# yxtay/glove-tensorflow

Hardware: AMD Instinct MI355X
Metric: co-occurrence nonzeros/sec (higher is better)
Workload: dtype f32; 1 GPU; zipf_v400k_d300; V=400000, d=300, optimizer=Adagrad, batch_size_per_gpu=1048576, global_batch=1048576, nnz_per_gpu=25000000, chunk_cap=32, parallelism=single GPU, index=dealt

## Files before the change

### glove-tensorflow_amd/csrc/glove_epoch.hip

```cpp
#include "glove_common.h"

#include <type_traits>

namespace glove {

constexpr int kCsThreads = 256;
constexpr int kCsWaves = kCsThreads / 64;
constexpr int kCsMaxDigits = 2048;
constexpr int kCsMaxBits = 11;

struct CsGeom {
    int64_t n;
    int ntiles;
    int nd[2], db[2];
    int stride;
    uint32_t *count, *offs;
    uint32_t *tot;
};

template <int E, class Job>
__global__ __launch_bounds__(kCsThreads) void csort_hist(Job job, CsGeom g)
{
    __shared__ int hist[kCsMaxDigits];
    const int side = blockIdx.y, nd = g.nd[side], db = g.db[side];
    for (int i = threadIdx.x; i < nd; i += kCsThreads) hist[i] = 0;
    __syncthreads();
    const int lane = threadIdx.x & 63, wave = threadIdx.x >> 6;
    const int64_t base = ((int64_t)blockIdx.x * kCsWaves + wave) * (64 * E);
    __shared__ uint32_t walk[Job::kSeats ? E * kCsThreads : 1];
    if (Job::kSeats) {
        int cnt = 0;
#pragma unroll
        for (int j = 0; j < E; ++j) {
            const int64_t i = base + j * 64 + lane;
            if (i < g.n) { walk[j * kCsThreads + threadIdx.x] = job.position(side, i); cnt = j + 1; }
        }
        int j = 0;
        uint32_t x = cnt > 0 ? walk[threadIdx.x] : 0u;
        while (j < cnt) {
            x = job.seat_once(x);
            if (job.seated(x)) {
                walk[j * kCsThreads + threadIdx.x] = x;
                ++j;
                if (j < cnt) x = walk[j * kCsThreads + threadIdx.x];
            }
        }
    }
#pragma unroll 4
    for (int j = 0; j < E; ++j) {
        const int64_t i = base + j * 64 + lane;
        const bool valid = i < g.n;
        int digit = 0;
        if (Job::kSeats) { if (valid) digit = job.digit_of_seat(side, i, walk[j * kCsThreads + threadIdx.x]); }
        else if (valid) digit = job.digit(side, i);
        const unsigned long long peers = digit_peers(digit, db, valid);
        if (valid && lane == __ffsll((long long)peers) - 1) atomicAdd(&hist[digit], __popcll(peers));
    }
    __syncthreads();
    uint32_t *out = g.count + (size_t)side * g.stride * g.ntiles + blockIdx.x;
    for (int i = threadIdx.x; i < nd; i += kCsThreads) out[(size_t)i * g.ntiles] = (uint32_t)hist[i];
}

__device__ inline int block_excl_scan(int v, int *wtot , int &total)
{
    const int lane = threadIdx.x & 63, wave = threadIdx.x >> 6;
    int incl = v;
#pragma unroll
    for (int dlt = 1; dlt < 64; dlt <<= 1) {
        const int o = __shfl_up(incl, dlt, 64);
        if (lane >= dlt) incl += o;
    }
    __syncthreads();
    if (lane == 63) wtot[wave] = incl;
    __syncthreads();
    int start = incl - v;
    total = 0;
#pragma unroll
    for (int wv = 0; wv < kCsWaves; ++wv) {
        if (wv < wave) start += wtot[wv];
        total += wtot[wv];
    }
    return start;
}

__global__ __launch_bounds__(kCsThreads) void csort_scan(CsGeom g)
{
    __shared__ int wtot[kCsWaves];
    const int side = blockIdx.y, d = blockIdx.x;
    if (d >= g.nd[side]) return;
    const uint32_t *row = g.count + ((size_t)side * g.stride + d) * g.ntiles;
    uint32_t *out = g.offs + ((size_t)side * g.stride + d) * g.ntiles;
    constexpr int kPer = 8;
    int carry = 0;
    for (int base = 0; base < g.ntiles; base += kCsThreads * kPer) {
        int v[kPer], s = 0;
#pragma unroll
        for (int k = 0; k < kPer; ++k) {
            const int t = base + threadIdx.x * kPer + k;
            v[k] = t < g.ntiles ? (int)row[t] : 0;
            s += v[k];
        }
        int total;
        int run = carry + block_excl_scan(s, wtot, total);
#pragma unroll
        for (int k = 0; k < kPer; ++k) {
            const int t = base + threadIdx.x * kPer + k;
            if (t < g.ntiles) out[t] = (uint32_t)run;
            run += v[k];
        }
        carry += total;
    }
    if (threadIdx.x == 0) g.tot[(size_t)side * g.stride + d] = (uint32_t)carry;
}

template <int E, class Job>
__global__ __launch_bounds__(kCsThreads) void csort_scatter(Job job, CsGeom g)
{
    using Item = typename Job::Item;
    constexpr int T = kCsThreads * E;
    extern __shared__ __attribute__((aligned(16))) unsigned char cs_smem[];
    const int side = blockIdx.y, nd = g.nd[side], db = g.db[side];
    Item *stage = reinterpret_cast<Item *>(cs_smem);
    uint16_t *sdig = reinterpret_cast<uint16_t *>(stage + T);
    int *wcnt = reinterpret_cast<int *>(sdig + T);
    int *gbase = wcnt + kCsWaves * nd;
    int *tstart = gbase + nd;
    __shared__ int wtot[kCsWaves];
    const int lane = threadIdx.x & 63, wave = threadIdx.x >> 6;
    const int64_t tile0 = (int64_t)blockIdx.x * T;
    const int64_t base = tile0 + (int64_t)wave * (64 * E);
    Item it[E];
    int digit[E], rank[E];
#pragma unroll
    for (int j = 0; j < E; ++j) {
        const int64_t i = base + j * 64 + lane;
        digit[j] = 0;
        if (i < g.n) digit[j] = job.load(side, i, it[j]);
    }
    int *mine = wcnt + wave * nd;
    for (int i = lane; i < nd; i += 64) mine[i] = 0;
#pragma unroll
    for (int j = 0; j < E; ++j) {
// ... 443 lines not shown
```

### glove-tensorflow_amd/csrc/glove_plan.hip

```cpp
#include "glove_common.h"

#include <cstring>

namespace glove {

constexpr int kSmallPlanMax = 4096;
int plan_build_small(const int32_t *row, const int32_t *col, const float *w, const float *y, int64_t B, int32_t V,
                     const PlanSet &set, int n, hipStream_t st);

constexpr int kSortThreads = 256;
constexpr int kSortWaves = kSortThreads / 64;
constexpr int kMaxDigits = 256;
constexpr int kWalk = 16;

struct SortSide {
    const int32_t *keys;
    const int32_t *vals;
    int32_t clean_below;
    int32_t *out_keys, *out_vals;
    int32_t *sorted_keys;
    const int32_t *other;
    int32_t other_below;
    int32_t *partner;
    float *w_out, *y_out;
    int32_t *where;
};

struct SortPass {
    SortSide s[2];
    const float *w, *y;
    int4 *pairs;
    int64_t n;
    int shift, db;
    int ntiles;
    uint16_t *count;
    int tile_stride;
    int32_t *mapped;
};

__device__ inline void block_store_sum(int v, int32_t *out)
{
    __shared__ int part[kSortWaves];
    v = wave_sum_int(v);
    if ((threadIdx.x & 63) == 0) part[threadIdx.x >> 6] = v;
    __syncthreads();
    if (threadIdx.x == 0) {
        int s = 0;
        for (int wv = 0; wv < kSortWaves; ++wv) s += part[wv];
        *out = s;
    }
}

template <int E>
__device__ inline void sort_load_keys(const SortSide &sd, int64_t n, int64_t base, int32_t (&key)[E], int &mapped)
{
    const int lane = threadIdx.x & 63;
#pragma unroll
    for (int j = 0; j < E; ++j) {
        const int64_t i = base + j * 64 + lane;
        int32_t k = 0;
        if (i < n) {
            k = sd.keys[i];
            if (sd.clean_below > 0 && (uint32_t)k >= (uint32_t)sd.clean_below) { k = 0; ++mapped; }
        }
        key[j] = k;
    }
}

struct SortPassSet { SortPass b[kPlanSetMax]; };
__device__ inline const SortPass &pick(const SortPass &a) { return a; }
__device__ inline const SortPass &pick(const SortPassSet &a) { return a.b[blockIdx.z]; }

template <int E, class Args>
__global__ __launch_bounds__(kSortThreads) void radix_hist(Args args)
{
    const SortPass &in = pick(args);
    static_assert(kSortThreads == kMaxDigits, "one thread per digit zeroes and stores the histogram");
    __shared__ int hist[kMaxDigits];
    const int side = blockIdx.y;
    const SortSide &sd = in.s[side];
    const int nd = 1 << in.db, lane = threadIdx.x & 63, wave = threadIdx.x >> 6;
    hist[threadIdx.x] = 0;
    __syncthreads();
    const int64_t base = ((int64_t)blockIdx.x * kSortWaves + wave) * (64 * E);
// ... 72 lines not shown
    int all = 0, earlier = 0;
    const int me = blockIdx.x;
    for (int q0 = 0; q0 < nq; q0 += kWalk) {
        if (q0 > 0) {
#pragma unroll
            for (int x = 0; x < kWalk; ++x) cw[x] = rowp[q0 + x < nq ? q0 + x : 0];
        }
#pragma unroll
        for (int x = 0; x < kWalk; ++x) {
            const uint32_t wd[4] = {cw[x].x, cw[x].y, cw[x].z, cw[x].w};
#pragma unroll
            for (int h = 0; h < 8; ++h) {
                const int t = (q0 + x) * 8 + h;
                const int c = (int)((wd[h >> 1] >> (16 * (h & 1))) & 0xffffu);
                all += (q0 + x < nq && t < in.ntiles) ? c : 0;
                earlier += (q0 + x < nq && t < me) ? c : 0;
            }
        }
    }
    if ((int)threadIdx.x >= nd) all = earlier = 0;
    int incl = all;
#pragma unroll
    for (int dlt = 1; dlt < 64; dlt <<= 1) {
        const int o = __shfl_up(incl, dlt, 64);
        if (lane >= dlt) incl += o;
    }
    if (lane == 63) scan_red[wave] = incl;
    __syncthreads();
    int start = incl - all + earlier;
    for (int wv = 0; wv < wave; ++wv) start += scan_red[wv];
    if ((int)threadIdx.x < nd) {
        int run = start;
#pragma unroll
        for (int wv = 0; wv < kSortWaves; ++wv) {
            const int c = wcnt[wv][threadIdx.x];
            wcnt[wv][threadIdx.x] = run;
            run += c;
        }
    }
    __syncthreads();
#pragma unroll
    for (int j = 0; j < E; ++j) {
        const int64_t i = base + j * 64 + lane;
        if (i >= in.n) continue;
        const int digit = (key[j] >> in.shift) & (nd - 1);
        const int dest = wcnt[wave][digit] + rank[j];
        const int32_t p = val[j];
        if (!LAST) {
            sd.out_keys[dest] = key[j];
            sd.out_vals[dest] = p;
        } else {
            sd.sorted_keys[dest] = key[j];
            int32_t o = g_id[j];
            if ((uint32_t)o >= (uint32_t)sd.other_below) o = 0;
            sd.partner[dest] = o;
            sd.w_out[dest] = g_w[j];
            sd.y_out[dest] = g_y[j];
            if (sd.where) { if (side == 0) sd.where[p] = dest; else sd.where[dest] = p; }
        }
    }
}


#define SIDE(x) (side ? x[1] : x[0])

constexpr int kTileThreads = 256;
constexpr int kTilePer = 8;
constexpr int kTile = kTileThreads * kTilePer;

struct SideKeys { const int32_t *keys[2]; };
struct SideOut {
    int32_t *chunk_id[2], *chunk_start[2], *uniq_slot[2];
    int32_t *counts;
    int32_t *uniq_rec[2];
    const int64_t *tile_re;
    int32_t *heavy;
    int heavy_chunks, cap_heavy;
    int2 *chunk_aux[2];
    uint32_t *mark[2];
    int mark_words[2];
    uint32_t *chunk_hw[2];
};

__device__ inline void tile_flags(const int32_t *__restrict__ keys, int64_t B, int64_t begin, int32_t chunk_cap,
                                  int64_t first_run_start, unsigned (&flag)[kTilePer], int &nu, int &nc, int64_t *lds_rs)
{
    const int64_t k0 = begin + (int64_t)threadIdx.x * kTilePer;
    int32_t key[kTilePer + 1];
    key[0] = (k0 > 0 && k0 <= B) ? keys[k0 - 1] : -1;
#pragma unroll
    for (int i = 0; i < kTilePer; ++i) key[i + 1] = (k0 + i < B) ? keys[k0 + i] : -1;
    int64_t my_last_start = -1;
#pragma unroll
    for (int i = 0; i < kTilePer; ++i) {
        const int64_t k = k0 + i;
        if (k < B && (k == 0 || key[i + 1] != key[i])) my_last_start = k;
    }
    const int lane = threadIdx.x & 63, wave = threadIdx.x >> 6;
    int64_t incl = my_last_start;
#pragma unroll
    for (int dlt = 1; dlt < 64; dlt <<= 1) {
        const int64_t o = __shfl_up(incl, dlt, 64);
        if (lane >= dlt) incl = o > incl ? o : incl;
    }
    if (lane == 63) lds_rs[wave] = incl;
    __syncthreads();
    int64_t carry = first_run_start;
    for (int wv = 0; wv < wave; ++wv) carry = lds_rs[wv] > carry ? lds_rs[wv] : carry;
    int64_t prev = __shfl_up(incl, 1, 64);
    if (lane == 0) prev = -1;
    int64_t run_start = prev > carry ? prev : carry;
    __syncthreads();
    nu = nc = 0;
#pragma unroll
    for (int i = 0; i < kTilePer; ++i) {
        const int64_t k = k0 + i;
        flag[i] = 0;
        if (k >= B) continue;
        const bool uniq = (k == 0 || key[i + 1] != key[i]);
        if (uniq) run_start = k;
        const bool chunk = uniq || ((int)(k - run_start) % chunk_cap == 0);
        flag[i] = (chunk ? 1u : 0u) | (uniq ? 2u : 0u);
        nu += uniq;
        nc += chunk;
    }
}

__device__ inline int64_t run_start_of(const int32_t *__restrict__ keys, int64_t pos)
{
    const int lane = threadIdx.x & 63;
    const int32_t key = keys[pos];
    int64_t lo = 0, hi = pos;
    if (pos > 0) {
        const int64_t q = pos - 1 - lane;
        const bool other = q >= 0 && keys[q] != key;
        const unsigned long long m = __ballot(other);
        if (m != 0) return pos - (__ffsll((long long)m) - 1);
        if (pos < 64) return 0;
        hi = pos - 64;
    }
    while (lo < hi) {
        const int64_t n = hi - lo, step = (n + 63) / 64;
        int64_t q = lo + step * lane;
        if (q > hi - 1) q = hi - 1;
        const bool ge = keys[q] >= key;
        const unsigned long long m = __ballot(ge);
        if (m == 0) {
            lo = __shfl(q, 63, 64) + 1;
            continue;
        }
        const int first = __ffsll((long long)m) - 1;
        const int64_t q_first = __shfl(q, first, 64);
        const int64_t q_before = __shfl(q, first > 0 ? first - 1 : 0, 64);
        lo = first == 0 ? lo : q_before + 1;
        hi = first == 0 ? lo : q_first;
    }
    return lo;
}

__device__ inline int64_t run_end_of(const int32_t *__restrict__ keys, int64_t B, int64_t pos)
{
    const int lane = threadIdx.x & 63;
    const int32_t key = keys[pos];
    int64_t lo = pos + 1, hi = B;
    {
        const int64_t q = pos + 1 + lane;
        const bool other = q < B && keys[q] != key;
        const unsigned long long m = __ballot(other);
        if (m != 0) return pos + 1 + (__ffsll((long long)m) - 1);
        if (pos + 65 >= B) return B;
        lo = pos + 65;
    }
    while (lo < hi) {
        const int64_t n = hi - lo, step = (n + 63) / 64;
        int64_t q = lo + step * lane;
        if (q > hi - 1) q = hi - 1;
        const bool gt = keys[q] > key;
        const unsigned long long m = __ballot(gt);
        if (m == 0) {
            lo = __shfl(q, 63, 64) + 1;
            continue;
        }
        const int first = __ffsll((long long)m) - 1;
        const int64_t q_first = __shfl(q, first, 64);
        const int64_t q_before = __shfl(q, first > 0 ? first - 1 : 0, 64);
        lo = first == 0 ? lo : q_before + 1;
        hi = first == 0 ? lo : q_first;
    }
    return lo;
}

struct TileExtra {
    int64_t *tile_re;
    int32_t *counts;
    const int32_t *mapped;
    int n_mapped;
    const int32_t *c_orig;
    const int32_t *rpos;
    int32_t *c_perm, *r_to_c;
};

struct SideCopy {
    const int32_t *p_src[2]; const float *w_src[2], *y_src[2];
    int32_t *p_dst[2]; float *w_dst[2], *y_dst[2];
};

struct SideOne {
    SideKeys sk;
    int64_t *tile_rs;
    int2 *tile_sums;
    TileExtra ex;
    SideOut out;
    SideCopy cp;
};
struct SideSet { SideOne b[kPlanSetMax]; };
__device__ inline const SideOne &pick(const SideOne &a) { return a; }
__device__ inline const SideOne &pick(const SideSet &a) { return a.b[blockIdx.z]; }

struct SortedSrc { const int32_t *id[2], *partner[2]; const float *w[2], *y[2]; };
struct SortedWs { char *base; size_t per_batch, tile_rs, tile_re, tile_sums, aux0, aux1; };
struct SideDev {
    const glove_plan *plans;
    SortedSrc src;
    SortedWs ws;
    int64_t B;
    int ntiles;
    int32_t V;
};
__device__ inline SideOne pick(const SideDev &a)
{
    const glove_plan &pl = a.plans[blockIdx.z];
    const size_t at = (size_t)blockIdx.z * (size_t)a.B;
    char *w = a.ws.base + (size_t)blockIdx.z * a.ws.per_batch;
    SideOne o;
    o.sk = SideKeys{{a.src.id[0] + at, a.src.id[1] + at}};
    o.tile_rs = reinterpret_cast<int64_t *>(w + a.ws.tile_rs);
    o.tile_sums = reinterpret_cast<int2 *>(w + a.ws.tile_sums);
    int64_t *tile_re = reinterpret_cast<int64_t *>(w + a.ws.tile_re);
    int2 *aux0 = reinterpret_cast<int2 *>(w + a.ws.aux0), *aux1 = reinterpret_cast<int2 *>(w + a.ws.aux1);
    o.ex = TileExtra{tile_re, pl.counts, nullptr, 0, nullptr, nullptr, nullptr, nullptr};
    o.out = SideOut{{pl.r_chunk_id, pl.c_chunk_id}, {pl.r_chunk_start, pl.c_chunk_start}, {pl.r_uniq_slot, pl.c_uniq_slot},
                    pl.counts, {pl.r_uniq_rec, pl.c_uniq_rec}, tile_re, pl.heavy, pl.heavy_chunks, pl.cap_heavy,
                    {pl.r_crec ? aux0 : nullptr, pl.r_crec ? aux1 : nullptr},
                    {pl.r_mark, pl.c_mark}, {((pl.V_row > 0 ? pl.V_row : a.V) + 31) / 32, (a.V + 31) / 32},
                    {pl.r_chunk_hw, pl.c_chunk_hw}};
    o.cp = SideCopy{{a.src.partner[0] + at, a.src.partner[1] + at}, {a.src.w[0] + at, a.src.w[1] + at}, {a.src.y[0] + at, a.src.y[1] + at},
                    {pl.r_partner, pl.c_partner}, {pl.r_w, pl.c_w}, {pl.r_y, pl.c_y}};
    return o;
}

template <class Args>
__global__ __launch_bounds__(kTileThreads) void side_tiles(Args args, int64_t B, int32_t chunk_cap, int ntiles)
{
    const SideOne &one = pick(args);
    const SideKeys &sk = one.sk;
    int64_t *__restrict__ tile_rs = one.tile_rs;
    int2 *__restrict__ tile_sums = one.tile_sums;
    const TileExtra &ex = one.ex;
    __shared__ int64_t lds_rs[kTileThreads / 64 + 1];
    __shared__ int red[2][kTileThreads / 64];
    const int side = blockIdx.y, t = blockIdx.x;
    const int32_t *keys = SIDE(sk.keys);
    const int64_t begin = (int64_t)t * kTile;
    if (SIDE(one.out.mark)) {
        uint32_t *mk = SIDE(one.out.mark);
        const int words = SIDE(one.out.mark_words);
        for (int i = t * kTileThreads + (int)threadIdx.x; i < words; i += ntiles * kTileThreads) mk[i] = 0u;
    }
    if (SIDE(one.cp.p_dst)) {
        const SideCopy &cp = one.cp;
        for (int64_t k = begin + threadIdx.x; k < begin + kTile && k < B; k += kTileThreads) {
            SIDE(cp.p_dst)[k] = SIDE(cp.p_src)[k];
            SIDE(cp.w_dst)[k] = SIDE(cp.w_src)[k];
            SIDE(cp.y_dst)[k] = SIDE(cp.y_src)[k];
        }
    }
    if (side == 1 && ex.c_perm) {
        const int64_t q0 = begin + (int64_t)threadIdx.x * kTilePer;
        int32_t o[kTilePer], rp[kTilePer];
#pragma unroll
        for (int i = 0; i < kTilePer; ++i) o[i] = q0 + i < B ? ex.c_orig[q0 + i] : 0;
#pragma unroll
        for (int i = 0; i < kTilePer; ++i) rp[i] = ex.rpos[o[i]];
#pragma unroll
        for (int i = 0; i < kTilePer; ++i) {
            if (q0 + i >= B) continue;
            ex.c_perm[q0 + i] = rp[i];
            ex.r_to_c[rp[i]] = (int32_t)(q0 + i);
        }
    }
    if (threadIdx.x < 64) {
        const int64_t r = begin > 0 ? run_start_of(keys, begin) : 0;
        if (threadIdx.x == 0) lds_rs[kTileThreads / 64] = r;
    } else if (threadIdx.x < 128) {
        const int64_t end = begin + kTile < B ? begin + kTile : B;
        const int64_t r = end < B ? run_end_of(keys, B, end - 1) : B;
        if (threadIdx.x == 64) ex.tile_re[(size_t)side * ntiles + t] = r;
    }
    __syncthreads();
    const int64_t frs = lds_rs[kTileThreads / 64];
    unsigned flag[kTilePer];
    int nu, nc;
    tile_flags(keys, B, begin, chunk_cap, frs, flag, nu, nc, lds_rs);
    nu = wave_sum_int(nu);
    nc = wave_sum_int(nc);
    if ((threadIdx.x & 63) == 0) { red[0][threadIdx.x >> 6] = nu; red[1][threadIdx.x >> 6] = nc; }
    __syncthreads();
    if (threadIdx.x == 0) {
        int su = 0, sc = 0;
        for (int wv = 0; wv < kTileThreads / 64; ++wv) { su += red[0][wv]; sc += red[1][wv]; }
        tile_sums[(size_t)side * ntiles + t] = make_int2(su, sc);
        tile_rs[(size_t)side * ntiles + t] = frs;
    }
    if (t == 0 && side == 0) {
        int v = 0;
        for (int i = threadIdx.x; i < ex.n_mapped; i += kTileThreads) v += ex.mapped[i];
        v = wave_sum_int(v);
        __syncthreads();
        if ((threadIdx.x & 63) == 0) red[0][threadIdx.x >> 6] = v;
        __syncthreads();
        if (threadIdx.x == 0) {
            int total = 0;
            for (int wv = 0; wv < kTileThreads / 64; ++wv) total += red[0][wv];
            ex.counts[5] = total;
            ex.counts[4] = ex.counts[6] = ex.counts[7] = 0;
        }
    }
}

template <class Args>
__global__ __launch_bounds__(kTileThreads) void side_emit(Args args, int64_t B, int32_t chunk_cap, int ntiles)
{
    const SideOne &one = pick(args);
    const SideKeys &sk = one.sk;
    const int64_t *__restrict__ tile_rs = one.tile_rs;
    const int2 *__restrict__ tile_sums = one.tile_sums;
    const SideOut &out = one.out;
    __shared__ int64_t lds_rs[kTileThreads / 64 + 1];
    __shared__ int64_t lds_open[kTileThreads / 64];
    __shared__ int red[2][kTileThreads / 64];
    __shared__ int wave_tot[2][kTileThreads / 64];
    const int side = blockIdx.y, t = blockIdx.x;
    const int32_t *keys = SIDE(sk.keys);
    const int64_t begin = (int64_t)t * kTile;
    int pu = 0, pc = 0;
    for (int i = threadIdx.x; i < t; i += kTileThreads) {
        const int2 v = tile_sums[(size_t)side * ntiles + i];
        pu += v.x;
        pc += v.y;
    }
    pu = wave_sum_int(pu);
    pc = wave_sum_int(pc);
    if ((threadIdx.x & 63) == 0) { red[0][threadIdx.x >> 6] = pu; red[1][threadIdx.x >> 6] = pc; }
    __syncthreads();
    int base_u = 0, base_c = 0;
    for (int wv = 0; wv < kTileThreads / 64; ++wv) { base_u += red[0][wv]; base_c += red[1][wv]; }
    unsigned flag[kTilePer];
    int nu, nc;
    tile_flags(keys, B, begin, chunk_cap, tile_rs[(size_t)side * ntiles + t], flag, nu, nc, lds_rs);
    const int lane = threadIdx.x & 63, wave = threadIdx.x >> 6;
    int iu = nu, ic = nc;
#pragma unroll
    for (int dlt = 1; dlt < 64; dlt <<= 1) {
        const int ou = __shfl_up(iu, dlt, 64), oc = __shfl_up(ic, dlt, 64);
        if (lane >= dlt) { iu += ou; ic += oc; }
    }
    if (lane == 63) { wave_tot[0][wave] = iu; wave_tot[1][wave] = ic; }
    __syncthreads();
    int ui = base_u + iu - nu, ci = base_c + ic - nc;
    for (int wv = 0; wv < wave; ++wv) { ui += wave_tot[0][wv]; ci += wave_tot[1][wv]; }
    const int64_t k0 = begin + (int64_t)threadIdx.x * kTilePer;
    int32_t *chunk_id = SIDE(out.chunk_id), *chunk_start = SIDE(out.chunk_start), *uniq_slot = SIDE(out.uniq_slot);
    int open_ui[kTilePer], open_ci[kTilePer];
    int64_t my_first_open = INT64_MAX;
#pragma unroll
    for (int i = kTilePer - 1; i >= 0; --i)
        if (flag[i] & 2u) my_first_open = k0 + i;
#pragma unroll
    for (int i = 0; i < kTilePer; ++i) {
        const int64_t k = k0 + i;
        open_ui[i] = ui;
        open_ci[i] = ci;
        if (flag[i] & 2u) uniq_slot[ui++] = ci;
        if (flag[i] & 1u) { chunk_id[ci] = keys[k]; chunk_start[ci] = (int32_t)k; ++ci; }
        if (k == B - 1) {
            chunk_start[ci] = (int32_t)B;
            uniq_slot[ui] = ci;
            out.counts[2 * side] = ci;
            out.counts[2 * side + 1] = ui;
        }
    }
    int64_t sfx = my_first_open;
#pragma unroll
    for (int dlt = 1; dlt < 64; dlt <<= 1) {
        const int64_t o = __shfl_down(sfx, dlt, 64);
        if (lane + dlt < 64) sfx = o < sfx ? o : sfx;
    }
    if (lane == 0) lds_open[wave] = sfx;
    __syncthreads();
    int64_t next_open = out.tile_re[(size_t)side * ntiles + t];
    for (int wv = kTileThreads / 64 - 1; wv > wave; --wv) next_open = lds_open[wv] < next_open ? lds_open[wv] : next_open;
    int64_t right = __shfl_down(sfx, 1, 64);
    if (lane == 63) right = INT64_MAX;
    next_open = right < next_open ? right : next_open;
    int2 *aux = SIDE(out.chunk_aux);
#pragma unroll
    for (int i = kTilePer - 1; i >= 0; --i) {
        if (!(flag[i] & 1u)) continue;
        const int64_t k = k0 + i;
        const int pairs = (int)(next_open - k), chunks = (pairs + chunk_cap - 1) / chunk_cap;
        if (aux || SIDE(out.chunk_hw)) {
            const bool opens = (flag[i] & 2u) != 0;
            const uint32_t hw = (uint32_t)(chunks - 1) | (opens ? 0x80000000u : 0u);
            if (aux) aux[open_ci[i]] = make_int2(opens ? open_ui[i] : open_ui[i] - 1, (int)hw);
            if (SIDE(out.chunk_hw)) SIDE(out.chunk_hw)[open_ci[i]] = hw;
        }
        if (!(flag[i] & 2u)) continue;
        reinterpret_cast<int4 *>(SIDE(out.uniq_rec))[open_ui[i]] = make_int4(keys[k], open_ci[i], chunks, pairs);
        if (SIDE(out.mark)) atomicOr(SIDE(out.mark) + (keys[k] >> 5), 1u << (keys[k] & 31));
        if (chunks > out.heavy_chunks) {
            const int slot = atomicAdd(out.counts + 4, 1);
            if (slot < out.cap_heavy) out.heavy[slot] = (side << 30) | open_ui[i];
        }
        next_open = k;
    }
}

struct RecordArgs {
    const int32_t *uniq_slot[2];
    const int32_t *chunk_id[2], *chunk_start[2], *partner[2];
    const float *w[2], *y[2];
    int32_t *crec[2];
    const int2 *chunk_aux[2];
    int header_in_record;
};
struct RecordOne { RecordArgs a; const int32_t *counts; };
struct RecordSet { RecordOne b[kPlanSetMax]; };
__device__ inline const RecordOne &pick(const RecordOne &a) { return a; }
__device__ inline const RecordOne &pick(const RecordSet &a) { return a.b[blockIdx.z]; }
struct RecordDev { SideDev d; };
__device__ inline RecordOne pick(const RecordDev &r)
{
    const SideDev &a = r.d;
    const glove_plan &pl = a.plans[blockIdx.z];
    const size_t at = (size_t)blockIdx.z * (size_t)a.B;
    char *w = a.ws.base + (size_t)blockIdx.z * a.ws.per_batch;
    RecordOne o;
    o.a = RecordArgs{{pl.r_uniq_slot, pl.c_uniq_slot}, {pl.r_chunk_id, pl.c_chunk_id}, {pl.r_chunk_start, pl.c_chunk_start},
                     {a.src.partner[0] + at, a.src.partner[1] + at}, {a.src.w[0] + at, a.src.w[1] + at}, {a.src.y[0] + at, a.src.y[1] + at},
                     {pl.r_crec, pl.c_crec},
                     {reinterpret_cast<const int2 *>(w + a.ws.aux0), reinterpret_cast<const int2 *>(w + a.ws.aux1)}, 0};
    o.counts = pl.counts;
    return o;
}

typedef int v4i_t __attribute__((ext_vector_type(4)));

template <class Args>
__global__ __launch_bounds__(kBlock) void fill_records(Args args, int capP, int nt)
{
    const RecordOne &rone = pick(args);
    const RecordArgs &a = rone.a;
    const int32_t *__restrict__ counts = rone.counts;
    const int side = blockIdx.y;
    const int n_chunks = counts[2 * side];
    const int32_t *chunk_id = SIDE(a.chunk_id), *chunk_start = SIDE(a.chunk_start), *partner = SIDE(a.partner);
    const float *w = SIDE(a.w), *y = SIDE(a.y);
    const int2 *aux = SIDE(a.chunk_aux);
    const int sq = rec_stride_q(capP);
    const int lane = threadIdx.x & 63, g = lane & 7, oct = lane >> 3;
    const int j0 = (int)((blockIdx.x * (kBlock / 64) + (threadIdx.x >> 6)) * 32);
    if (j0 >= n_chunks) return;
    const int jl = j0 + lane < n_chunks ? j0 + lane : n_chunks;
    const int cs = lane <= 32 ? chunk_start[jl] : 0;
    constexpr int kStage = 384;
    __shared__ int32_t st_p[kBlock / 64][kStage];
    __shared__ float st_w[kBlock / 64][kStage], st_y[kBlock / 64][kStage];
    const int wv = threadIdx.x >> 6;
    const int p0 = __shfl(cs, 0, 64);
    const int last = n_chunks - j0 < 32 ? n_chunks - j0 : 32;
    const int span = __shfl(cs, last, 64) - p0;
    const bool staged = span <= kStage;
    if (staged) {
        for (int i = lane; i < span; i += 64) {
            st_p[wv][i] = partner[p0 + i];
            st_w[wv][i] = w[p0 + i];
            st_y[wv][i] = y[p0 + i];
        }
    }
    int32_t cid = 0;
    int2 ax = make_int2(0, 0);
    if (lane < 32 && j0 + lane < n_chunks) {
        cid = chunk_id[j0 + lane];
        if (aux) {
            ax = aux[j0 + lane];
        } else if (a.header_in_record) {
            ax = *reinterpret_cast<const int2 *>(SIDE(a.crec) + (size_t)(j0 + lane) * sq * 4 + 2);
        } else {
            const int j = j0 + lane;
            const int32_t *slot = SIDE(a.uniq_slot);
            int lo = 0, hi = counts[2 * side + 1];
            while (hi - lo > 1) {
                const int mid = (lo + hi) >> 1;
                if (slot[mid] <= j) lo = mid; else hi = mid;
            }
            ax = make_int2(lo, (int)((uint32_t)(slot[lo + 1] - 1 - j) | (slot[lo] == j ? 0x80000000u : 0u)));
        }
    }
// ... 139 lines not shown
            SortPass &in = set.b[j];
            in = fin[j];
            for (int sd = 0; sd < 2; ++sd) {
                if (p > 0) {
                    in.s[sd].keys = pw[j].keys[sd][(p - 1) & 1];
                    in.s[sd].vals = pw[j].vals[sd][(p - 1) & 1];
                    in.s[sd].clean_below = 0;
                }
                in.s[sd].out_keys = pw[j].keys[sd][p & 1];
                in.s[sd].out_vals = pw[j].vals[sd][p & 1];
            }
            in.n = B;
            in.shift = p * db;
            in.db = db;
            in.ntiles = pw[j].sort_tiles;
            in.count = pw[j].count;
            in.tile_stride = pw[j].tile_stride;
            in.mapped = pw[j].mapped;
        }
        const dim3 grid(pw[0].sort_tiles, 2, nb);
        if (nb == 1) {
            hipLaunchKernelGGL((radix_hist<E, SortPass>), grid, dim3(kSortThreads), 0, st, set.b[0]);
            if (p < P - 1) hipLaunchKernelGGL((radix_scatter<E, false, SortPass>), grid, dim3(kSortThreads), 0, st, set.b[0]);
            else hipLaunchKernelGGL((radix_scatter<E, true, SortPass>), grid, dim3(kSortThreads), 0, st, set.b[0]);
        } else {
            hipLaunchKernelGGL((radix_hist<E, SortPassSet>), grid, dim3(kSortThreads), 0, st, set);
            if (p < P - 1) hipLaunchKernelGGL((radix_scatter<E, false, SortPassSet>), grid, dim3(kSortThreads), 0, st, set);
            else hipLaunchKernelGGL((radix_scatter<E, true, SortPassSet>), grid, dim3(kSortThreads), 0, st, set);
        }
    }
}

#define HIP_TRY(expr) do { hipError_t e_ = (expr); if (e_ != hipSuccess) return (int)e_; } while (0)

static int build_tiled_set(const int32_t *row, const int32_t *col, const float *w, const float *y, int64_t B, int32_t V,
                           const glove_plan *const *plans, int nb, void *ws, size_t ws_bytes, hipStream_t st)
{
    const size_t per = carve_plan_ws(nullptr, B).bytes;
    if (per * (size_t)nb > ws_bytes) return GLOVE_E_WORKSPACE;
    PlanWs pw[kPlanSetMax];
    SortPass fin[kPlanSetMax];
    const int bits = ceil_log2(V);
    for (int j = 0; j < nb; ++j) {
        const glove_plan *plan = plans[j];
        pw[j] = carve_plan_ws((char *)ws + per * j, B);
        const int32_t Vr = plan->V_row > 0 ? plan->V_row : V;
        const size_t off = (size_t)j * B;
        SortPass &f = fin[j];
        f = SortPass{};
        f.w = w + off; f.y = y + off; f.pairs = pw[j].pairs;
        SortSide &rs = f.s[0], &cs = f.s[1];
        rs.keys = row + off; rs.vals = nullptr; rs.clean_below = Vr;
        rs.sorted_keys = pw[j].row_sorted; rs.other = col + off; rs.other_below = V;
        rs.partner = plan->r_partner; rs.w_out = plan->r_w; rs.y_out = plan->r_y; rs.where = plan->c_perm ? pw[j].rpos : nullptr;
        cs.keys = col + off; cs.vals = nullptr; cs.clean_below = V;
        cs.sorted_keys = pw[j].col_sorted; cs.other = row + off; cs.other_below = Vr;
        cs.partner = plan->c_partner; cs.w_out = plan->c_w; cs.y_out = plan->c_y; cs.where = plan->c_perm ? pw[j].c_orig : nullptr;
    }
    if (pw[0].sort_e == 4) launch_sorts<4>(fin, pw, nb, B, bits, st);
    else if (pw[0].sort_e == 8) launch_sorts<8>(fin, pw, nb, B, bits, st);
    else launch_sorts<16>(fin, pw, nb, B, bits, st);

    SideSet ss;
    const int2 *aux_r[kPlanSetMax], *aux_c[kPlanSetMax];
    for (int j = 0; j < nb; ++j) {
        const glove_plan *plan = plans[j];
        ss.b[j].sk = SideKeys{{pw[j].row_sorted, pw[j].col_sorted}};
        ss.b[j].tile_rs = pw[j].tile_rs;
        ss.b[j].tile_sums = pw[j].tile_sums;
        ss.b[j].out = SideOut{{plan->r_chunk_id, plan->c_chunk_id}, {plan->r_chunk_start, plan->c_chunk_start},
                            {plan->r_uniq_slot, plan->c_uniq_slot}, plan->counts, {plan->r_uniq_rec, plan->c_uniq_rec},
                            (const int64_t *)pw[j].tile_re, plan->heavy, plan->heavy_chunks, plan->cap_heavy,
                            {plan->r_crec ? pw[j].chunk_aux[0] : nullptr, plan->r_crec ? pw[j].chunk_aux[1] : nullptr},
                            {plan->r_mark, plan->c_mark}, {(Vr_of(plan, V) + 31) / 32, (V + 31) / 32},
                            {plan->r_chunk_hw, plan->c_chunk_hw}};
        ss.b[j].cp = SideCopy{};
        ss.b[j].ex = TileExtra{pw[j].tile_re, plan->counts, (const int32_t *)pw[j].mapped, 2 * pw[j].sort_tiles,
                             (const int32_t *)pw[j].c_orig, (const int32_t *)pw[j].rpos, plan->c_perm, plan->r_to_c};
        aux_r[j] = pw[j].chunk_aux[0];
        aux_c[j] = pw[j].chunk_aux[1];
    }
    const dim3 grid(pw[0].ntiles, 2, nb);
    if (nb == 1) {
        hipLaunchKernelGGL(side_tiles<SideOne>, grid, dim3(kTileThreads), 0, st, ss.b[0], B, plans[0]->chunk_cap, pw[0].ntiles);
        hipLaunchKernelGGL(side_emit<SideOne>, grid, dim3(kTileThreads), 0, st, ss.b[0], B, plans[0]->chunk_cap, pw[0].ntiles);
    } else {
        hipLaunchKernelGGL(side_tiles<SideSet>, grid, dim3(kTileThreads), 0, st, ss, B, plans[0]->chunk_cap, pw[0].ntiles);
        hipLaunchKernelGGL(side_emit<SideSet>, grid, dim3(kTileThreads), 0, st, ss, B, plans[0]->chunk_cap, pw[0].ntiles);
    }
    if (plans[0]->r_crec) return launch_fill_records_set(plans, nb, st, aux_r, aux_c);
    return (int)hipGetLastError();
}

}

using namespace glove;

extern "C" {

size_t glove_plan_workspace_bytes(int64_t B, int32_t V)
{
    (void)V;
    if (B < 0) return 0;
    return carve_plan_ws(nullptr, B).bytes;
}

static int check_plan_for_build(const glove_plan *plan, int64_t B, int32_t V)
{
    if (!plan->r_partner || !plan->r_w || !plan->r_y || !plan->r_chunk_id || !plan->r_chunk_start || !plan->r_uniq_slot ||
        !plan->c_w || !plan->c_y || !plan->r_uniq_rec || !plan->c_uniq_rec || !plan->c_partner || !plan->c_chunk_id || !plan->c_chunk_start || !plan->c_uniq_slot)
        return GLOVE_E_BADARG;
    if (!plan->heavy || plan->heavy_chunks < 1 ||
        plan->cap_heavy < 2 * B / ((int64_t)plan->heavy_chunks * plan->chunk_cap) + 2)
        return GLOVE_E_WORKSPACE;
    if (plan->cap_chunks < B || plan->cap_uniq < (B < V ? B : V)) return GLOVE_E_WORKSPACE;
    if ((plan->r_crec == nullptr) != (plan->c_crec == nullptr)) return GLOVE_E_BADARG;
    if ((plan->r_to_c == nullptr) != (plan->c_perm == nullptr)) return GLOVE_E_BADARG;
    if ((plan->r_mark == nullptr) != (plan->c_mark == nullptr)) return GLOVE_E_BADARG;
    if ((plan->r_chunk_hw == nullptr) != (plan->c_chunk_hw == nullptr)) return GLOVE_E_BADARG;
    return 0;
}

int glove_plan_build(const int32_t *row, const int32_t *col, const float *w, const float *y, int64_t B, int32_t V,
                     const glove_plan *plan, void *ws, size_t ws_bytes, void *stream)
{
    if (!plan || !ws || B < 0 || V <= 0 || plan->chunk_cap <= 0 || plan->B != B || !plan->counts) return GLOVE_E_BADARG;
    hipStream_t st = (hipStream_t)stream;
    if (B == 0) {
        HIP_TRY(zero_words(plan->counts, 8, st));
        return 0;
    }
    if (!row || !col || !w || !y) return GLOVE_E_BADARG;
    if (int rc = check_plan_for_build(plan, B, V)) return rc;
    if (B <= kSmallPlanMax) {
        PlanSet set;
        set.p[0] = *plan;
        if (int rc = plan_build_small(row, col, w, y, B, V, set, 1, st)) return rc;
        return plan->r_crec ? launch_fill_records(plan, st, true) : 0;
    }
    return build_tiled_set(row, col, w, y, B, V, &plan, 1, ws, ws_bytes, st);
}

static SortedWs carve_sorted_ws(void *ws, int64_t B, int *ntiles_out)
{
    SortedWs s;
    size_t off = 0;
    auto take = [&](size_t bytes) { const size_t q = off; off += align_up(bytes, 256); return q; };
    const size_t n = (size_t)(B > 0 ? B : 1);
    const int ntiles = (int)((n + kTile - 1) / kTile);
    s.base = (char *)ws;
    s.tile_rs = take((size_t)2 * ntiles * 8);
    s.tile_re = take((size_t)2 * ntiles * 8);
    s.tile_sums = take((size_t)2 * ntiles * 8);
    s.aux0 = take(n * 8);
    s.aux1 = take(n * 8);
    s.per_batch = off;
    if (ntiles_out) *ntiles_out = ntiles;
    return s;
}

size_t glove_plan_sorted_workspace_bytes(int64_t B, int32_t n_batches)
{
    if (B < 0 || n_batches < 0) return 0;
    return carve_sorted_ws(nullptr, B, nullptr).per_batch * (size_t)n_batches;
}

int32_t glove_plan_chunk_bound(int64_t B, int32_t cap_uniq, int32_t chunk_cap)
{
    if (B < 0 || cap_uniq < 0 || chunk_cap <= 0) return 0;
    const int64_t bound = (int64_t)cap_uniq + B / chunk_cap + 1;
    return (int32_t)(bound < B ? bound : B);
}

int glove_plan_build_sorted(const glove_pairs *row_side, const glove_pairs *col_side, int64_t first_pair, int64_t B,
                            int32_t n_batches, int32_t V, const glove_plan *plans, const glove_plan *plans_dev, void *ws,
                            size_t ws_bytes, void *stream)
{
    if (!row_side || !col_side || !plans || !plans_dev || first_pair < 0 || B <= 0 || n_batches < 0 || V <= 0) return GLOVE_E_BADARG;
    if (n_batches == 0) return 0;
    if (!row_side->id || !row_side->partner || !row_side->w || !row_side->y || !col_side->id || !col_side->partner || !col_side->w ||
        !col_side->y || !ws)
        return GLOVE_E_BADARG;
    int64_t most = 1;
    for (int j = 0; j < n_batches; ++j) {
        const glove_plan *p = plans + j;
        if (p->B != B || p->chunk_cap <= 0 || p->chunk_cap != plans[0].chunk_cap || !p->counts) return GLOVE_E_BADARG;
        if ((p->r_crec == nullptr) != (plans[0].r_crec == nullptr) || (p->r_crec == nullptr) != (p->c_crec == nullptr)) return GLOVE_E_BADARG;
        if (!p->r_chunk_id || !p->r_chunk_start || !p->r_uniq_slot || !p->r_uniq_rec || !p->c_chunk_id || !p->c_chunk_start ||
            !p->c_uniq_slot || !p->c_uniq_rec)
            return GLOVE_E_BADARG;
        const bool own = p->r_partner || p->r_w || p->r_y || p->c_partner || p->c_w || p->c_y;
        if (own && (!p->r_partner || !p->r_w || !p->r_y || !p->c_partner || !p->c_w || !p->c_y)) return GLOVE_E_BADARG;
        if (!own && !p->r_crec && !p->r_chunk_hw) return GLOVE_E_BADARG;
        if (p->c_perm || p->r_to_c) return GLOVE_E_BADARG;
        if ((p->r_mark == nullptr) != (p->c_mark == nullptr)) return GLOVE_E_BADARG;
        if ((p->r_chunk_hw == nullptr) != (p->c_chunk_hw == nullptr)) return GLOVE_E_BADARG;
        if (!p->heavy || p->heavy_chunks < 1 || p->cap_heavy < 2 * B / ((int64_t)p->heavy_chunks * p->chunk_cap) + 2) return GLOVE_E_WORKSPACE;
        if (p->cap_uniq < (B < V ? B : V)) return GLOVE_E_WORKSPACE;
        if (p->cap_chunks < glove_plan_chunk_bound(B, p->cap_uniq, p->chunk_cap)) return GLOVE_E_WORKSPACE;
        const int64_t mr = most_chunks(p, true), mc = most_chunks(p, false);
        most = mr > most ? mr : most;
        most = mc > most ? mc : most;
    }
    SideDev sd;
    sd.plans = plans_dev;
    sd.src = SortedSrc{{row_side->id + first_pair, col_side->id + first_pair}, {row_side->partner + first_pair, col_side->partner + first_pair},
                       {row_side->w + first_pair, col_side->w + first_pair}, {row_side->y + first_pair, col_side->y + first_pair}};
    sd.ws = carve_sorted_ws(ws, B, &sd.ntiles);
    sd.B = B;
    sd.V = V;
    if (sd.ws.per_batch * (size_t)n_batches > ws_bytes) return GLOVE_E_WORKSPACE;
    hipStream_t st = (hipStream_t)stream;
    const int32_t cap = plans[0].chunk_cap;
    for (int z0 = 0; z0 < n_batches; z0 += 65535) {
        const int nz = n_batches - z0 < 65535 ? n_batches - z0 : 65535;
        SideDev part = sd;
        part.plans = plans_dev + z0;
        part.ws.base = sd.ws.base + (size_t)z0 * sd.ws.per_batch;
        for (int x = 0; x < 2; ++x) {
            part.src.id[x] += (size_t)z0 * B; part.src.partner[x] += (size_t)z0 * B;
            part.src.w[x] += (size_t)z0 * B; part.src.y[x] += (size_t)z0 * B;
        }
        const dim3 grid(sd.ntiles, 2, nz);
        hipLaunchKernelGGL(side_tiles<SideDev>, grid, dim3(kTileThreads), 0, st, part, B, cap, sd.ntiles);
        hipLaunchKernelGGL(side_emit<SideDev>, grid, dim3(kTileThreads), 0, st, part, B, cap, sd.ntiles);
        if (plans[0].r_crec) {
            const int64_t per_block = (kBlock / 64) * 32;
            const int64_t nb = (most + per_block - 1) / per_block;
            hipLaunchKernelGGL(fill_records<RecordDev>, dim3((unsigned)(nb < 1 ? 1 : nb), 2, nz), dim3(kBlock), 0, st, RecordDev{part}, rec_cap(cap), B >= 262144 ? 1 : 0);
        }
    }
    return (int)hipGetLastError();
}

int glove_plan_fill_records(const glove_plan *plan, void *stream)
{
    if (!plan || !plan->r_crec || !plan->c_crec || !plan->counts || plan->chunk_cap <= 0) return GLOVE_E_BADARG;
    if (plan->B == 0) return 0;
    if (!plan->r_uniq_slot || !plan->c_uniq_slot) return GLOVE_E_BADARG;
    if (!plan->r_chunk_id || !plan->r_chunk_start || !plan->r_partner || !plan->r_w || !plan->r_y || !plan->c_chunk_id ||
        !plan->c_chunk_start || !plan->c_partner || !plan->c_w || !plan->c_y)
        return GLOVE_E_BADARG;
    return launch_fill_records(plan, (hipStream_t)stream);
}

}
```

Before: 1.866 billion nonzeros/s.

## Privatize small-radix histograms and streamline plan tile scan kernels

When a counting-sort pass has few digits, the histogram kernel now keeps 32 lane-indexed copies per digit in LDS and adds plain atomics to them, reducing them at the end instead of doing match-peer aggregation. The plan tile kernels load keys with 16-byte vector loads for full aligned tiles. They move run-start arithmetic to 32-bit tile-local offsets and replace the per-element modulo by chunk_cap with a running counter plus a precomputed magic-number divide. They also pack the unique and chunk counts into one int for a single wave reduction and scan, and drop a barrier by reordering the prefix-sum reads. The packing assumes per-tile counts fit in 16 bits, and the vector path adds a second template instantiation and more register pressure.

```diff
diff --git a/glove-tensorflow_amd/csrc/glove_epoch.hip b/glove-tensorflow_amd/csrc/glove_epoch.hip
--- a/glove-tensorflow_amd/csrc/glove_epoch.hip
+++ b/glove-tensorflow_amd/csrc/glove_epoch.hip
@@ -8,6 +8,9 @@
 constexpr int kCsWaves = kCsThreads / 64;
 constexpr int kCsMaxDigits = 2048;
 constexpr int kCsMaxBits = 11;
+constexpr int kCsFewDigits = 64;
+constexpr int kCsCopies = 32;
+static_assert(kCsFewDigits * kCsCopies <= kCsMaxDigits, "the copies share the histogram's LDS");
 
 struct CsGeom {
     int64_t n;
@@ -23,7 +26,8 @@
 {
     __shared__ int hist[kCsMaxDigits];
     const int side = blockIdx.y, nd = g.nd[side], db = g.db[side];
-    for (int i = threadIdx.x; i < nd; i += kCsThreads) hist[i] = 0;
+    const bool few = nd <= kCsFewDigits;
+    for (int i = threadIdx.x; i < (few ? nd * kCsCopies : nd); i += kCsThreads) hist[i] = 0;
     __syncthreads();
     const int lane = threadIdx.x & 63, wave = threadIdx.x >> 6;
     const int64_t base = ((int64_t)blockIdx.x * kCsWaves + wave) * (64 * E);
@@ -53,11 +57,28 @@
         int digit = 0;
         if (Job::kSeats) { if (valid) digit = job.digit_of_seat(side, i, walk[j * kCsThreads + threadIdx.x]); }
         else if (valid) digit = job.digit(side, i);
+        if (few) {
+            if (valid) atomicAdd(&hist[digit * kCsCopies + (lane & (kCsCopies - 1))], 1);
+            continue;
+        }
         const unsigned long long peers = digit_peers(digit, db, valid);
         if (valid && lane == __ffsll((long long)peers) - 1) atomicAdd(&hist[digit], __popcll(peers));
     }
     __syncthreads();
     uint32_t *out = g.count + (size_t)side * g.stride * g.ntiles + blockIdx.x;
+    if (few) {
+        static_assert(kCsFewDigits * 4 == kCsThreads && kCsCopies == 32, "four threads per digit, eight copies per thread");
+        const int d = threadIdx.x >> 2, part = threadIdx.x & 3;
+        int v = 0;
+        if (d < nd) {
+#pragma unroll
+            for (int r = 0; r < kCsCopies / 4; ++r) v += hist[d * kCsCopies + part * (kCsCopies / 4) + r];
+        }
+        v += __shfl_xor(v, 1, 64);
+        v += __shfl_xor(v, 2, 64);
+        if (d < nd && part == 0) out[(size_t)d * g.ntiles] = (uint32_t)v;
+        return;
+    }
     for (int i = threadIdx.x; i < nd; i += kCsThreads) out[(size_t)i * g.ntiles] = (uint32_t)hist[i];
 }
 
diff --git a/glove-tensorflow_amd/csrc/glove_plan.hip b/glove-tensorflow_amd/csrc/glove_plan.hip
--- a/glove-tensorflow_amd/csrc/glove_plan.hip
+++ b/glove-tensorflow_amd/csrc/glove_plan.hip
@@ -1,5 +1,6 @@
 #include "glove_common.h"
 
+#include <climits>
 #include <cstring>
 
 namespace glove {
@@ -238,47 +239,78 @@
     uint32_t *chunk_hw[2];
 };
 
-__device__ inline void tile_flags(const int32_t *__restrict__ keys, int64_t B, int64_t begin, int32_t chunk_cap,
-                                  int64_t first_run_start, unsigned (&flag)[kTilePer], int &nu, int &nc, int64_t *lds_rs)
-{
-    const int64_t k0 = begin + (int64_t)threadIdx.x * kTilePer;
-    int32_t key[kTilePer + 1];
-    key[0] = (k0 > 0 && k0 <= B) ? keys[k0 - 1] : -1;
-#pragma unroll
-    for (int i = 0; i < kTilePer; ++i) key[i + 1] = (k0 + i < B) ? keys[k0 + i] : -1;
-    int64_t my_last_start = -1;
+struct CapDiv { uint32_t m; int shift; };
+static CapDiv cap_div(int32_t d)
+{
+    int l = 0;
+    while ((1ll << l) < d) ++l;
+    const uint64_t p = 1ull << (31 + l);
+    return CapDiv{(uint32_t)((p + (uint64_t)d - 1) / (uint64_t)d), 31 + l};
+}
+__device__ inline int div_cap(int a, CapDiv cd) { return (int)(((uint64_t)(uint32_t)a * cd.m) >> cd.shift); }
+
+__device__ inline bool tile_whole(const int32_t *keys, int64_t B, int64_t begin)
+{
+    return begin + kTile <= B && (reinterpret_cast<uintptr_t>(keys + begin) & 15u) == 0;
+}
+
+template <bool WHOLE>
+__device__ inline void tile_keys(const int32_t *__restrict__ keys, int64_t B, int64_t k0, int32_t (&key)[kTilePer + 1])
+{
+    static_assert(kTilePer == 8, "two 16-byte loads per thread");
+    if (WHOLE) {
+        const int32_t front = keys[k0 > 0 ? k0 - 1 : 0];
+        const int4 a = *reinterpret_cast<const int4 *>(keys + k0), b = *reinterpret_cast<const int4 *>(keys + k0 + 4);
+        key[0] = k0 > 0 ? front : -1;
+        key[1] = a.x; key[2] = a.y; key[3] = a.z; key[4] = a.w;
+        key[5] = b.x; key[6] = b.y; key[7] = b.z; key[8] = b.w;
+    } else {
+        key[0] = (k0 > 0 && k0 <= B) ? keys[k0 - 1] : -1;
+#pragma unroll
+        for (int i = 0; i < kTilePer; ++i) key[i + 1] = (k0 + i < B) ? keys[k0 + i] : -1;
+    }
+}
+
+__device__ inline void tile_flags(const int32_t (&key)[kTilePer + 1], int64_t B, int64_t begin, int32_t chunk_cap, CapDiv cd,
+                                  int first_run_start, unsigned (&flag)[kTilePer], int &nu, int &nc, int *lds_rs)
+{
+    const int l0 = (int)threadIdx.x * kTilePer;
+    const int left = (int)(B - begin < kTile ? B - begin : kTile);
+    int my_last_start = INT_MIN;
 #pragma unroll
     for (int i = 0; i < kTilePer; ++i) {
-        const int64_t k = k0 + i;
-        if (k < B && (k == 0 || key[i + 1] != key[i])) my_last_start = k;
+        const int l = l0 + i;
+        if (l < left && ((begin == 0 && l == 0) || key[i + 1] != key[i])) my_last_start = l;
     }
     const int lane = threadIdx.x & 63, wave = threadIdx.x >> 6;
-    int64_t incl = my_last_start;
+    int incl = my_last_start;
 #pragma unroll
     for (int dlt = 1; dlt < 64; dlt <<= 1) {
-        const int64_t o = __shfl_up(incl, dlt, 64);
+        const int o = __shfl_up(incl, dlt, 64);
         if (lane >= dlt) incl = o > incl ? o : incl;
     }
     if (lane == 63) lds_rs[wave] = incl;
+    int prev = __shfl_up(incl, 1, 64);
+    if (lane == 0) prev = INT_MIN;
     __syncthreads();
-    int64_t carry = first_run_start;
+    int carry = first_run_start;
     for (int wv = 0; wv < wave; ++wv) carry = lds_rs[wv] > carry ? lds_rs[wv] : carry;
-    int64_t prev = __shfl_up(incl, 1, 64);
-    if (lane == 0) prev = -1;
-    int64_t run_start = prev > carry ? prev : carry;
-    __syncthreads();
+    int run_start = prev > carry ? prev : carry;
+    int behind = l0 < left ? l0 - run_start : 0;
+    behind -= div_cap(behind, cd) * chunk_cap;
     nu = nc = 0;
 #pragma unroll
     for (int i = 0; i < kTilePer; ++i) {
-        const int64_t k = k0 + i;
+        const int l = l0 + i;
         flag[i] = 0;
-        if (k >= B) continue;
-        const bool uniq = (k == 0 || key[i + 1] != key[i]);
-        if (uniq) run_start = k;
-        const bool chunk = uniq || ((int)(k - run_start) % chunk_cap == 0);
+        if (l >= left) continue;
+        const bool uniq = ((begin == 0 && l == 0) || key[i + 1] != key[i]);
+        if (uniq) behind = 0;
+        const bool chunk = behind == 0;
         flag[i] = (chunk ? 1u : 0u) | (uniq ? 2u : 0u);
         nu += uniq;
         nc += chunk;
+        if (++behind == chunk_cap) behind = 0;
     }
 }
 
@@ -405,19 +437,21 @@
     return o;
 }
 
-template <class Args>
-__global__ __launch_bounds__(kTileThreads) void side_tiles(Args args, int64_t B, int32_t chunk_cap, int ntiles)
-{
-    const SideOne &one = pick(args);
+template <bool WHOLE>
+__device__ inline void side_tiles_body(const SideOne &one, int64_t B, int32_t chunk_cap, CapDiv cd, int ntiles)
+{
     const SideKeys &sk = one.sk;
     int64_t *__restrict__ tile_rs = one.tile_rs;
     int2 *__restrict__ tile_sums = one.tile_sums;
     const TileExtra &ex = one.ex;
-    __shared__ int64_t lds_rs[kTileThreads / 64 + 1];
+    __shared__ int lds_rs[kTileThreads / 64];
+    __shared__ int64_t lds_frs;
     __shared__ int red[2][kTileThreads / 64];
     const int side = blockIdx.y, t = blockIdx.x;
     const int32_t *keys = SIDE(sk.keys);
     const int64_t begin = (int64_t)t * kTile;
+    int32_t key[kTilePer + 1];
+    tile_keys<WHOLE>(keys, B, begin + (int64_t)threadIdx.x * kTilePer, key);
     if (SIDE(one.out.mark)) {
         uint32_t *mk = SIDE(one.out.mark);
         const int words = SIDE(one.out.mark_words);
@@ -447,19 +481,20 @@
     }
     if (threadIdx.x < 64) {
         const int64_t r = begin > 0 ? run_start_of(keys, begin) : 0;
-        if (threadIdx.x == 0) lds_rs[kTileThreads / 64] = r;
+        if (threadIdx.x == 0) lds_frs = r;
     } else if (threadIdx.x < 128) {
         const int64_t end = begin + kTile < B ? begin + kTile : B;
         const int64_t r = end < B ? run_end_of(keys, B, end - 1) : B;
         if (threadIdx.x == 64) ex.tile_re[(size_t)side * ntiles + t] = r;
     }
     __syncthreads();
-    const int64_t frs = lds_rs[kTileThreads / 64];
+    const int64_t frs = lds_frs;
     unsigned flag[kTilePer];
     int nu, nc;
-    tile_flags(keys, B, begin, chunk_cap, frs, flag, nu, nc, lds_rs);
-    nu = wave_sum_int(nu);
-    nc = wave_sum_int(nc);
+    tile_flags(key, B, begin, chunk_cap, cd, (int)(frs - begin), flag, nu, nc, lds_rs);
+    nu = wave_sum_int(nu | nc << 16);
+    nc = nu >> 16;
+    nu &= 0xffff;
     if ((threadIdx.x & 63) == 0) { red[0][threadIdx.x >> 6] = nu; red[1][threadIdx.x >> 6] = nc; }
     __syncthreads();
     if (threadIdx.x == 0) {
@@ -485,22 +520,36 @@
 }
 
 template <class Args>
-__global__ __launch_bounds__(kTileThreads) void side_emit(Args args, int64_t B, int32_t chunk_cap, int ntiles)
+__global__ __launch_bounds__(kTileThreads) void side_tiles(Args args, int64_t B, int32_t chunk_cap, CapDiv cd, int ntiles)
 {
     const SideOne &one = pick(args);
+    const int side = blockIdx.y;
+    if (tile_whole(SIDE(one.sk.keys), B, (int64_t)blockIdx.x * kTile)) side_tiles_body<true>(one, B, chunk_cap, cd, ntiles);
+    else side_tiles_body<false>(one, B, chunk_cap, cd, ntiles);
+}
+
+template <bool WHOLE>
+__device__ inline void side_emit_body(const SideOne &one, int64_t B, int32_t chunk_cap, CapDiv cd, int ntiles)
+{
     const SideKeys &sk = one.sk;
     const int64_t *__restrict__ tile_rs = one.tile_rs;
     const int2 *__restrict__ tile_sums = one.tile_sums;
     const SideOut &out = one.out;
-    __shared__ int64_t lds_rs[kTileThreads / 64 + 1];
-    __shared__ int64_t lds_open[kTileThreads / 64];
+    __shared__ int lds_rs[kTileThreads / 64];
+    __shared__ int lds_open[kTileThreads / 64];
     __shared__ int red[2][kTileThreads / 64];
-    __shared__ int wave_tot[2][kTileThreads / 64];
+    __shared__ int wave_tot[kTileThreads / 64];
     const int side = blockIdx.y, t = blockIdx.x;
     const int32_t *keys = SIDE(sk.keys);
     const int64_t begin = (int64_t)t * kTile;
-    int pu = 0, pc = 0;
-    for (int i = threadIdx.x; i < t; i += kTileThreads) {
+    int32_t key[kTilePer + 1];
+    tile_keys<WHOLE>(keys, B, begin + (int64_t)threadIdx.x * kTilePer, key);
+    int2 s0 = make_int2(0, 0), s1 = make_int2(0, 0);
+    if ((int)threadIdx.x < t) s0 = tile_sums[(size_t)side * ntiles + threadIdx.x];
+    if ((int)threadIdx.x + kTileThreads < t) s1 = tile_sums[(size_t)side * ntiles + threadIdx.x + kTileThreads];
+    const int64_t frs = tile_rs[(size_t)side * ntiles + t], re = out.tile_re[(size_t)side * ntiles + t];
+    int pu = s0.x + s1.x, pc = s0.y + s1.y;
+    for (int i = threadIdx.x + 2 * kTileThreads; i < t; i += kTileThreads) {
         const int2 v = tile_sums[(size_t)side * ntiles + i];
         pu += v.x;
         pc += v.y;
@@ -508,63 +557,64 @@
     pu = wave_sum_int(pu);
     pc = wave_sum_int(pc);
     if ((threadIdx.x & 63) == 0) { red[0][threadIdx.x >> 6] = pu; red[1][threadIdx.x >> 6] = pc; }
-    __syncthreads();
+    unsigned flag[kTilePer];
+    int nu, nc;
+    tile_flags(key, B, begin, chunk_cap, cd, (int)(frs - begin), flag, nu, nc, lds_rs);
     int base_u = 0, base_c = 0;
     for (int wv = 0; wv < kTileThreads / 64; ++wv) { base_u += red[0][wv]; base_c += red[1][wv]; }
-    unsigned flag[kTilePer];
-    int nu, nc;
-    tile_flags(keys, B, begin, chunk_cap, tile_rs[(size_t)side * ntiles + t], flag, nu, nc, lds_rs);
     const int lane = threadIdx.x & 63, wave = threadIdx.x >> 6;
-    int iu = nu, ic = nc;
+    const int mine = nu | nc << 16;
+    int incl = mine;
 #pragma unroll
     for (int dlt = 1; dlt < 64; dlt <<= 1) {
-        const int ou = __shfl_up(iu, dlt, 64), oc = __shfl_up(ic, dlt, 64);
-        if (lane >= dlt) { iu += ou; ic += oc; }
-    }
-    if (lane == 63) { wave_tot[0][wave] = iu; wave_tot[1][wave] = ic; }
+        const int o = __shfl_up(incl, dlt, 64);
+        if (lane >= dlt) incl += o;
+    }
+    if (lane == 63) wave_tot[wave] = incl;
+    const int l0 = (int)threadIdx.x * kTilePer;
+    int my_first_open = INT_MAX;
+#pragma unroll
+    for (int i = kTilePer - 1; i >= 0; --i)
+        if (flag[i] & 2u) my_first_open = l0 + i;
+    int sfx = my_first_open;
+#pragma unroll
+    for (int dlt = 1; dlt < 64; dlt <<= 1) {
+        const int o = __shfl_down(sfx, dlt, 64);
+        if (lane + dlt < 64) sfx = o < sfx ? o : sfx;
+    }
+    if (lane == 0) lds_open[wave] = sfx;
     __syncthreads();
-    int ui = base_u + iu - nu, ci = base_c + ic - nc;
-    for (int wv = 0; wv < wave; ++wv) { ui += wave_tot[0][wv]; ci += wave_tot[1][wv]; }
-    const int64_t k0 = begin + (int64_t)threadIdx.x * kTilePer;
+    int before = incl - mine;
+    for (int wv = 0; wv < wave; ++wv) before += wave_tot[wv];
+    int ui = base_u + (before & 0xffff), ci = base_c + (before >> 16);
     int32_t *chunk_id = SIDE(out.chunk_id), *chunk_start = SIDE(out.chunk_start), *uniq_slot = SIDE(out.uniq_slot);
     int open_ui[kTilePer], open_ci[kTilePer];
-    int64_t my_first_open = INT64_MAX;
-#pragma unroll
-    for (int i = kTilePer - 1; i >= 0; --i)
-        if (flag[i] & 2u) my_first_open = k0 + i;
+    const int last = (int)(B - 1 - begin);
 #pragma unroll
     for (int i = 0; i < kTilePer; ++i) {
-        const int64_t k = k0 + i;
+        const int l = l0 + i;
         open_ui[i] = ui;
         open_ci[i] = ci;
         if (flag[i] & 2u) uniq_slot[ui++] = ci;
-        if (flag[i] & 1u) { chunk_id[ci] = keys[k]; chunk_start[ci] = (int32_t)k; ++ci; }
-        if (k == B - 1) {
+        if (flag[i] & 1u) { chunk_id[ci] = key[i + 1]; chunk_start[ci] = (int32_t)(begin + l); ++ci; }
+        if (l == last) {
             chunk_start[ci] = (int32_t)B;
             uniq_slot[ui] = ci;
             out.counts[2 * side] = ci;
             out.counts[2 * side + 1] = ui;
         }
     }
-    int64_t sfx = my_first_open;
-#pragma unroll
-    for (int dlt = 1; dlt < 64; dlt <<= 1) {
-        const int64_t o = __shfl_down(sfx, dlt, 64);
-        if (lane + dlt < 64) sfx = o < sfx ? o : sfx;
-    }
-    if (lane == 0) lds_open[wave] = sfx;
-    __syncthreads();
-    int64_t next_open = out.tile_re[(size_t)side * ntiles + t];
+    int next_open = (int)(re - begin);
     for (int wv = kTileThreads / 64 - 1; wv > wave; --wv) next_open = lds_open[wv] < next_open ? lds_open[wv] : next_open;
-    int64_t right = __shfl_down(sfx, 1, 64);
-    if (lane == 63) right = INT64_MAX;
+    int right = __shfl_down(sfx, 1, 64);
+    if (lane == 63) right = INT_MAX;
     next_open = right < next_open ? right : next_open;
     int2 *aux = SIDE(out.chunk_aux);
 #pragma unroll
     for (int i = kTilePer - 1; i >= 0; --i) {
         if (!(flag[i] & 1u)) continue;
-        const int64_t k = k0 + i;
-        const int pairs = (int)(next_open - k), chunks = (pairs + chunk_cap - 1) / chunk_cap;
+        const int l = l0 + i;
+        const int pairs = next_open - l, chunks = div_cap(pairs - 1, cd) + 1;
         if (aux || SIDE(out.chunk_hw)) {
             const bool opens = (flag[i] & 2u) != 0;
             const uint32_t hw = (uint32_t)(chunks - 1) | (opens ? 0x80000000u : 0u);
@@ -572,14 +622,23 @@
             if (SIDE(out.chunk_hw)) SIDE(out.chunk_hw)[open_ci[i]] = hw;
         }
         if (!(flag[i] & 2u)) continue;
-        reinterpret_cast<int4 *>(SIDE(out.uniq_rec))[open_ui[i]] = make_int4(keys[k], open_ci[i], chunks, pairs);
-        if (SIDE(out.mark)) atomicOr(SIDE(out.mark) + (keys[k] >> 5), 1u << (keys[k] & 31));
+        reinterpret_cast<int4 *>(SIDE(out.uniq_rec))[open_ui[i]] = make_int4(key[i + 1], open_ci[i], chunks, pairs);
+        if (SIDE(out.mark)) atomicOr(SIDE(out.mark) + (key[i + 1] >> 5), 1u << (key[i + 1] & 31));
         if (chunks > out.heavy_chunks) {
             const int slot = atomicAdd(out.counts + 4, 1);
             if (slot < out.cap_heavy) out.heavy[slot] = (side << 30) | open_ui[i];
         }
-        next_open = k;
-    }
+        next_open = l;
+    }
+}
+
+template <class Args>
+__global__ __launch_bounds__(kTileThreads) void side_emit(Args args, int64_t B, int32_t chunk_cap, CapDiv cd, int ntiles)
+{
+    const SideOne &one = pick(args);
+    const int side = blockIdx.y;
+    if (tile_whole(SIDE(one.sk.keys), B, (int64_t)blockIdx.x * kTile)) side_emit_body<true>(one, B, chunk_cap, cd, ntiles);
+    else side_emit_body<false>(one, B, chunk_cap, cd, ntiles);
 }
 
 struct RecordArgs {
@@ -885,11 +944,11 @@
     }
     const dim3 grid(pw[0].ntiles, 2, nb);
     if (nb == 1) {
-        hipLaunchKernelGGL(side_tiles<SideOne>, grid, dim3(kTileThreads), 0, st, ss.b[0], B, plans[0]->chunk_cap, pw[0].ntiles);
-        hipLaunchKernelGGL(side_emit<SideOne>, grid, dim3(kTileThreads), 0, st, ss.b[0], B, plans[0]->chunk_cap, pw[0].ntiles);
+        hipLaunchKernelGGL(side_tiles<SideOne>, grid, dim3(kTileThreads), 0, st, ss.b[0], B, plans[0]->chunk_cap, cap_div(plans[0]->chunk_cap), pw[0].ntiles);
+        hipLaunchKernelGGL(side_emit<SideOne>, grid, dim3(kTileThreads), 0, st, ss.b[0], B, plans[0]->chunk_cap, cap_div(plans[0]->chunk_cap), pw[0].ntiles);
     } else {
-        hipLaunchKernelGGL(side_tiles<SideSet>, grid, dim3(kTileThreads), 0, st, ss, B, plans[0]->chunk_cap, pw[0].ntiles);
-        hipLaunchKernelGGL(side_emit<SideSet>, grid, dim3(kTileThreads), 0, st, ss, B, plans[0]->chunk_cap, pw[0].ntiles);
+        hipLaunchKernelGGL(side_tiles<SideSet>, grid, dim3(kTileThreads), 0, st, ss, B, plans[0]->chunk_cap, cap_div(plans[0]->chunk_cap), pw[0].ntiles);
+        hipLaunchKernelGGL(side_emit<SideSet>, grid, dim3(kTileThreads), 0, st, ss, B, plans[0]->chunk_cap, cap_div(plans[0]->chunk_cap), pw[0].ntiles);
     }
     if (plans[0]->r_crec) return launch_fill_records_set(plans, nb, st, aux_r, aux_c);
     return (int)hipGetLastError();
@@ -1025,8 +1084,8 @@
             part.src.w[x] += (size_t)z0 * B; part.src.y[x] += (size_t)z0 * B;
         }
         const dim3 grid(sd.ntiles, 2, nz);
-        hipLaunchKernelGGL(side_tiles<SideDev>, grid, dim3(kTileThreads), 0, st, part, B, cap, sd.ntiles);
-        hipLaunchKernelGGL(side_emit<SideDev>, grid, dim3(kTileThreads), 0, st, part, B, cap, sd.ntiles);
+        hipLaunchKernelGGL(side_tiles<SideDev>, grid, dim3(kTileThreads), 0, st, part, B, cap, cap_div(cap), sd.ntiles);
+        hipLaunchKernelGGL(side_emit<SideDev>, grid, dim3(kTileThreads), 0, st, part, B, cap, cap_div(cap), sd.ntiles);
         if (plans[0].r_crec) {
             const int64_t per_block = (kBlock / 64) * 32;
             const int64_t nb = (most + per_block - 1) / per_block;
```

Result: no change. 1.894 billion nonzeros/s (median of 4 runs) (+1.5%).
